# mako443/Text2Pos-CVPR2022

Hardware: AMD Instinct MI355X
Metric: cells+queries encoded/sec and top-k retrieval QPS, 256-pt cells, 12k-cell DB (higher is better)
Workload: dtype f16x3 (fp32 operands split hi+lo into fp16, 3 f16 MFMAs, fp32 accumulate; fp32-class error) for the encoders / f64 MFMA for the ranking

## Files before the change

### include/t2p.h

```cpp
#ifndef T2P_H
#define T2P_H
#include <stddef.h>
#include <stdint.h>

#ifdef __cplusplus
extern "C" {
#endif

#define T2P_ABI_VERSION 31
#define T2P_DEFAULT_CHUNK_OBJECTS 65000
#define T2P_MAX_CHUNK_OBJECTS 65535
#define T2P_TUNING_MASK 0x5
#define T2P_E_ARG (-1)
#define T2P_E_WORKSPACE (-2)
#define T2P_E_UNSUPPORTED (-3)

typedef void* t2p_stream_t;

int t2p_abi_version(void);
const char* t2p_last_error(void);

typedef struct t2p_cell_weights {
    const float* sa_w1[3];
    const float* sa_b1[3];
    const float* sa_w2[3];
    const float* sa_b2[3];
    const float* ga_w1;
    const float* ga_b1;
    const float* ga_w2;
    const float* ga_b2;
    const float* lin1_w;
    const float* lin1_b;
    const float* lin2_w;
    const float* lin2_b;
    const float* pn_w;
    const float* pn_b;
    const float* col_w1;
    const float* col_b1;
    const float* col_w2;
    const float* col_b2;
    const float* pos_w1;
    const float* pos_b1;
    const float* pos_w2;
    const float* pos_b2;
    const float* merge_w;
// ... 221 lines not shown
```

### profiles/tail_rows_census.py

```python
#!/usr/bin/env python
import argparse
import os
import sys

import numpy as np

sys.path.insert(0, os.path.join(os.path.dirname(os.path.abspath(__file__)), ".."))

RADII = (0.2, 0.3, 0.4)
MAX_NBR = 32


def level(pos: np.ndarray, r: float):
    n_d = pos.shape[0]
    n_c = (n_d + 1) // 2
    r2 = np.float32(r) * np.float32(r)
    mind = np.full(n_d, np.inf, dtype=np.float32)
    fps = np.zeros(n_c, dtype=np.int64)
    cnt = np.zeros(n_c, dtype=np.int64)
    cur = 0
    for c in range(n_c):
        fps[c] = cur
        d = pos - pos[cur]
        d2 = (d[:, 0] * d[:, 0] + d[:, 1] * d[:, 1]) + d[:, 2] * d[:, 2]
        cnt[c] = min(int((d2 < r2).sum()), MAX_NBR)
        mind = np.minimum(mind, d2)
        cur = int(np.argmax(mind))
    return fps, cnt


def dedup_hits(pos: np.ndarray, rgb: np.ndarray, fps: np.ndarray, r: float) -> int:
    key = np.concatenate([pos, rgb], axis=1).view(np.uint32)
    _, first = np.unique(key, axis=0, return_index=True)
    orig = np.zeros(pos.shape[0], dtype=bool)
    orig[first] = True
    r2 = np.float32(r) * np.float32(r)
    kept = 0
    for c in fps:
        d = pos - pos[c]
        d2 = (d[:, 0] * d[:, 0] + d[:, 1] * d[:, 1]) + d[:, 2] * d[:, 2]
        hits = np.flatnonzero(d2 < r2)[:MAX_NBR]
        kept += int(orig[hits].sum())
    return kept


def main():
    ap = argparse.ArgumentParser(description=__doc__.split("\n")[0])
    ap.add_argument("--seed", type=int, default=20220002, help="bench.py's object stream")
    ap.add_argument("--objects", type=int, default=3000)
    args = ap.parse_args()
    from importlib import import_module
    S = import_module("text2pos-cvpr2022_amd.synthetic")
    xyz, rgb, _, _ = S.make_objects(args.seed, 0, args.objects)
    n = xyz.shape[0]
    rows = np.zeros(3)
    rows_dedup = 0.0
    with_tail = np.zeros(3)
    tail_cent = np.zeros(3)
    tail_rows = np.zeros(3)
    executed = np.zeros(3)
    cents = np.zeros(3)
    for o in range(n):
        pos = xyz[o].astype(np.float32)
        for l in range(3):
            fps, cnt = level(pos, RADII[l])
            n_c = fps.shape[0]
            tail = (fps == 0) & (np.arange(n_c) > 0)
            all_rows = cnt.sum() + n_c
            t_rows = cnt[tail].sum()
            rows[l] += all_rows
            cents[l] += n_c
            with_tail[l] += tail.any()
            tail_cent[l] += tail.sum()
            tail_rows[l] += t_rows
            executed[l] += all_rows - t_rows + (cnt[0] if tail.any() else 0)
            if l == 0:
                rows_dedup += dedup_hits(pos, rgb[o].astype(np.float32), fps, RADII[0]) + n_c
            pos = pos[fps]
    print(f"{n} objects of seed {args.seed}")
    print("level | rows/object | objects with a tail | tail centroids | tail rows (non-self) | rows/object, tail shared")
    for l in range(3):
        extra = f" ({rows_dedup / n:.0f} after point dedup)" if l == 0 else ""
        print(f"SA{l + 1}   | {rows[l] / n:8.0f}{extra} | {100 * with_tail[l] / n:5.1f} % | {100 * tail_cent[l] / cents[l]:5.1f} % | "
              f"{100 * tail_rows[l] / rows[l]:5.1f} % | {executed[l] / n:8.0f} ({100 * (executed[l] / rows[l] - 1):+.1f} %)")


if __name__ == "__main__":
    main()
```

### text2pos-cvpr2022_amd/csrc/api.hip

```cpp
#include <stdarg.h>
#include <stdlib.h>
#include <string.h>

#include <mutex>
#include <set>
#include <utility>

#include "../../include/t2p.h"
#include "t2p_common.h"

namespace t2p {

static thread_local char g_err[512] = "";

void set_error(const char* fmt, ...) {
    va_list ap;
    va_start(ap, fmt);
    vsnprintf(g_err, sizeof(g_err), fmt, ap);
    va_end(ap);
}

int num_cus() {
    static int cached = 0;
    if (cached == 0) {
// ... 960 lines not shown
    for (int l = 0; l < 3; l++) {
        gt.fps_idx[l] = fps_idx[l];
        gt.nbr[l] = nbr[l];
        gt.cnt[l] = cnt[l];
        gt.rows[l] = nullptr;
        gt.n_rows[l] = nullptr;
        gt.n_dense[l] = g.nd[l];
        gt.n_cent[l] = g.nc[l];
    }
    return launch_sample_group(xyz, n_obj, n_pts, radius_host, gt, (hipStream_t)stream);
}

int t2p_group_rows(const float* xyz, int64_t n_obj, int32_t n_pts, const float* radius_host, int32_t self_loops,
                   uint8_t* const* fps_idx, uint16_t* const* rows, uint16_t* const* n_rows, t2p_stream_t stream) {
    T2P_CHECK_ARG(xyz && radius_host && fps_idx && rows && n_rows, "group_rows: NULL argument");
    Geo g(n_pts);
    GroupTables gt{};
    gt.self_loops = self_loops ? 1 : 0;
    for (int l = 0; l < 3; l++) {
        T2P_CHECK_ARG(fps_idx[l] && rows[l] && n_rows[l], "group_rows: NULL table of level %d", l);
        gt.fps_idx[l] = fps_idx[l];
        gt.rows[l] = rows[l];
        gt.n_rows[l] = n_rows[l];
        gt.n_dense[l] = g.nd[l];
        gt.n_cent[l] = g.nc[l];
    }
    return launch_sample_group(xyz, n_obj, n_pts, radius_host, gt, (hipStream_t)stream);
}

int t2p_group_rows_shared(const float* xyz, int64_t n_obj, int32_t n_pts, const float* radius_host, int32_t self_loops,
                          int32_t share_mask, uint8_t* const* fps_idx, uint16_t* const* rows, uint16_t* const* n_rows,
                          t2p_stream_t stream) {
    T2P_CHECK_ARG(xyz && radius_host && fps_idx && rows && n_rows, "group_rows_shared: NULL argument");
    T2P_CHECK_ARG((share_mask & ~2) == 0, "group_rows_shared: share_mask=%#x (bit 1: SA level 2; no other level has a shared form)", share_mask);
    T2P_CHECK_ARG(share_mask == 0 || n_pts == 256, "group_rows_shared: shared lists exist for 256 points per object (n_pts = %d)", n_pts);
    Geo g(n_pts);
    GroupTables gt{};
    gt.self_loops = self_loops ? 1 : 0;
    for (int l = 0; l < 3; l++) {
        T2P_CHECK_ARG(fps_idx[l] && rows[l] && n_rows[l], "group_rows_shared: NULL table of level %d", l);
        gt.fps_idx[l] = fps_idx[l];
        gt.rows[l] = rows[l];
        gt.n_rows[l] = n_rows[l];
        gt.n_dense[l] = g.nd[l];
        gt.n_cent[l] = g.nc[l];
        gt.share_tail[l] = (share_mask >> l) & 1;
    }
    return launch_sample_group(xyz, n_obj, n_pts, radius_host, gt, (hipStream_t)stream);
}

int t2p_edge_counts(const uint16_t* rows, const uint16_t* n_rows, const int32_t* first_obj, int64_t n_obj, int32_t n_dense,
                    int32_t n_cent, int32_t self_loops, int32_t* counts, t2p_stream_t stream) {
    T2P_CHECK_ARG(n_obj >= 0 && (n_obj == 0 || (rows && n_rows && first_obj && counts)), "edge_counts: NULL argument");
    return launch_edge_counts(rows, n_rows, first_obj, n_obj, n_dense, n_cent, self_loops, counts, (hipStream_t)stream);
}

int t2p_edge_expand(const uint16_t* rows, const uint16_t* n_rows, const int32_t* first_obj, const int32_t* cent_ptr, int64_t n_obj,
                    int32_t n_dense, int32_t n_cent, int32_t self_loops, int32_t* src, int32_t* dst, t2p_stream_t stream) {
    T2P_CHECK_ARG(n_obj >= 0 && (n_obj == 0 || (rows && n_rows && first_obj && cent_ptr)), "edge_expand: NULL argument");
    return launch_edge_expand(rows, n_rows, first_obj, cent_ptr, n_obj, n_dense, n_cent, self_loops, src, dst, (hipStream_t)stream);
}

int t2p_pack_objects(const float* raw_xyz, const float* raw_rgb, const int32_t* obj_ptr, const int32_t* sample_idx,
                     const float* rot_cos_sin, int64_t n_obj, int32_t n_pts, float* xyz, float* rgb, float* center, float* mean_rgb,
                     t2p_stream_t stream) {
    T2P_CHECK_ARG(raw_xyz && raw_rgb && obj_ptr && sample_idx && xyz && rgb && center && mean_rgb, "pack_objects: NULL argument");
    T2P_CHECK_ARG(n_obj >= 0 && n_pts >= 1, "pack_objects: bad sizes");
// ... 53 lines not shown
```

### text2pos-cvpr2022_amd/csrc/sa_points.hip

```cpp
#ifndef T2P_PABL
#define T2P_PABL 0
#endif
#include "t2p_common.h"

namespace t2p {
namespace {

typedef uint32_t u32x4 __attribute__((ext_vector_type(4)));
typedef uint32_t u32x2 __attribute__((ext_vector_type(2)));
typedef float f32x2 __attribute__((ext_vector_type(2)));

#define MFMA16(a, b, c) __builtin_amdgcn_mfma_f32_32x32x16_f16(a, b, c, 0, 0, 0)
#define MFMA8(a, b, c) __builtin_amdgcn_mfma_f32_32x32x8f16(a, b, c, 0, 0, 0)

template <int NW>
struct PtsCfg {
    static constexpr int K = 32, N = 64, NC = 128, ND = 256, GS = 16;
    static constexpr int NT = 64 * NW;
    static constexpr int S16 = K / 16, NTW = N / 32;
    static constexpr int HS = GS / 2, NH = NC / HS;
    static constexpr int MAXR = NC * 33;
    static constexpr int LPR = 64 / HS;
    static constexpr int ACC_BYTES = GS * N * 4;
    static constexpr int PTS_BYTES = ND * 24;
    static constexpr int SELF_BYTES = GS * 24;
    static constexpr int CEN_BYTES = GS * 32;
    static constexpr int RING_BYTES = 4 * 64 * 2;
    static constexpr int WAVE_BYTES = ACC_BYTES + PTS_BYTES + SELF_BYTES + CEN_BYTES + 16 + 64 + RING_BYTES;
    static_assert(WAVE_BYTES % 16 == 0, "16-byte accesses");
    static constexpr size_t lds_bytes() { return (size_t)NW * WAVE_BYTES + 16 + N * 4; }
};

__device__ __forceinline__ float relu1(float v) {
    const int b = __float_as_int(v);
    return __int_as_float(b > 0 ? b : 0);
}
__device__ __forceinline__ void split2(float v0, float v1, uint32_t& hi, uint32_t& lo) {
    const fp16x2 hh = cvt_pk_f16(v0, v1);
    const fp16x2 ll = cvt_pk_f16(sub_half<0>(v0, hh), sub_half<1>(v1, hh));
    hi = __builtin_bit_cast(uint32_t, hh);
    lo = __builtin_bit_cast(uint32_t, ll);
}

template <int NW, int PARTS>
__global__ __launch_bounds__(64 * NW, (NW + 3) / 4) void k_sa_points(SaParams p) {
    using C = PtsCfg<NW>;
    static_assert(PARTS == 1 || (C::NH % PARTS == 0 && C::NH / PARTS >= 3), "a part is a whole number (>= 3: two open + one fetched ahead) of halves");
    constexpr int K = C::K, N = C::N, NC = C::NC;
    extern __shared__ __attribute__((aligned(16))) char lds[];
    const int tid = threadIdx.x, lane = tid & 63;
    const int wave = __builtin_amdgcn_readfirstlane(tid >> 6);
    const int h = lane >> 5, rr = lane & 31;
    const uint32_t acc_off = (uint32_t)(wave * C::WAVE_BYTES);
    const uint32_t pts_off = acc_off + C::ACC_BYTES;
    const uint32_t self_off = pts_off + C::PTS_BYTES;
    const uint32_t cen_off = self_off + C::SELF_BYTES;
    const uint32_t one_off = cen_off + C::CEN_BYTES;
    const uint32_t dst_off = one_off + 16;
    const uint32_t ring_off = dst_off + 64;
    if (lane == 0) *(f32x4*)(lds + one_off) = f32x4{1.f, 0.f, 0.f, 0.f};

    half8 w_hi[C::NTW][C::S16], w_lo[C::NTW][C::S16];
    {
        const uint4* wp = (const uint4*)p.W_x3;
        constexpr int PLANE_U4 = (N / 32) * C::S16 * 64;
#pragma unroll
        for (int nt = 0; nt < C::NTW; nt++)
#pragma unroll
            for (int s = 0; s < C::S16; s++) {
                uint4 pc[2][2];
#pragma unroll
                for (int hp = 0; hp < 2; hp++) {
                    const int kb = 16 * s + 8 * hp;
                    const int half_ = kb / (K / 2), step_ = (kb % (K / 2)) / 8;
                    const int idx = (((nt * C::S16 + step_) * 2 + half_) * 32) + rr;
                    pc[0][hp] = wp[idx];
                    pc[1][hp] = wp[PLANE_U4 + idx];
                }
                const u32x4 vh = h ? u32x4{pc[0][0].z, pc[0][0].w, pc[0][1].z, pc[0][1].w} : u32x4{pc[0][0].x, pc[0][0].y, pc[0][1].x, pc[0][1].y};
                const u32x4 vl = h ? u32x4{pc[1][0].z, pc[1][0].w, pc[1][1].z, pc[1][1].w} : u32x4{pc[1][0].x, pc[1][0].y, pc[1][1].x, pc[1][1].y};
                w_hi[nt][s] = __builtin_bit_cast(half8, vh);
                w_lo[nt][s] = __builtin_bit_cast(half8, vl);
            }
    }
    half4 w1_hi, w1_lo;
    {
// ... 6 lines not shown
        uint32_t hi0, lo0, hi1, lo1;
        split2(wv[0], wv[1], hi0, lo0);
        split2(wv[2], wv[3], hi1, lo1);
        w1_hi = __builtin_bit_cast(half4, u32x2{hi0, hi1});
        w1_lo = __builtin_bit_cast(half4, u32x2{lo0, lo1});
    }
    constexpr f32x16 kZero16 = {0.f, 0.f, 0.f, 0.f, 0.f, 0.f, 0.f, 0.f, 0.f, 0.f, 0.f, 0.f, 0.f, 0.f, 0.f, 0.f};

    const int cr = lane / C::LPR, cs = lane % C::LPR;
    constexpr int NPL = N / C::LPR;
    const uint32_t bias_off = (uint32_t)(NW * C::WAVE_BYTES + 16 + cs * NPL * 4);
    if (tid < N) *(float*)(lds + NW * C::WAVE_BYTES + 16 + tid * 4) = p.bias[tid];

    int gtop = 0;
    const int g_begin = p.bounds_ws[blockIdx.x], g_end = p.bounds_ws[blockIdx.x + 1];
    int* ctr = (int*)(lds + NW * C::WAVE_BYTES);
    if (tid == 0) *ctr = 0;
    __syncthreads();

    f32x4 pout[NPL / 4];
    float* pptr = nullptr;
    bool has_pout = false;
    for (;;) {
        int gi = 0;
        if (lane == 0) gi = atomicAdd(ctr, 1);
        gi = __builtin_amdgcn_readfirstlane(gi);
        const int g = g_begin + (PARTS > 1 ? gi / PARTS : gi);
        if (g >= g_end) break;
        constexpr int HP = C::NH / PARTS;
        const int hs = PARTS > 1 ? (gi % PARTS) * HP : 0;
        const int hend = hs + HP;
        int n = __builtin_amdgcn_readfirstlane((int)p.n_rows[g]);
        const uint16_t* list = p.rows + (int64_t)g * C::MAXR;
        if constexpr (PARTS > 1) {
            auto lower = [&](int target) -> int {
                if (target <= 0 || n <= 0) return 0;
                if (target >= NC) return n;
                const int step = (n + 63) >> 6;
                const int i0 = lane * step;
                const uint32_t c0 = i0 < n ? (((uint32_t)list[i0] >> 8) & 127u) : 255u;
                const unsigned long long ge = __ballot(c0 >= (uint32_t)target);
                const int fl = ge ? (int)__builtin_ctzll(ge) : 64;
                if (fl == 0) return 0;
                int hi = fl * step;
                hi = hi < n ? hi : n;
                const int base = (fl - 1) * step + 1;
                for (int b = base; b < hi; b += 64) {
                    const int i = b + lane;
                    const uint32_t c = i < hi ? (((uint32_t)list[i] >> 8) & 127u) : 255u;
                    const unsigned long long m = __ballot(c >= (uint32_t)target);
                    if (m) return b + (int)__builtin_ctzll(m);
                }
                return hi;
            };
            const int r_lo = __builtin_amdgcn_readfirstlane(lower(hs * C::HS));
            const int r_hi = __builtin_amdgcn_readfirstlane(lower(hend * C::HS));
            list += r_lo;
            n = r_hi - r_lo;
        }
        const int first = __builtin_amdgcn_readfirstlane(p.first[g]);
        const uint32_t sb0 = (uint32_t)(first * C::ND + (g - first) * NC);

        const int nwin = (n + 63) >> 6;
        auto load_win = [&](int w) -> uint32_t {
            int i = w * 64 + lane;
            i = i < n ? i : n - 1;
// ... 3 lines not shown
        auto ring_write = [&](int w, uint32_t v) { *(uint16_t*)(lds + ring_off + (((w & 3) * 64 + lane) * 2)) = (uint16_t)v; };
        auto ring_read = [&](int r) -> uint32_t {
            return (uint32_t) * (const uint16_t*)(lds + ring_off + (((r + rr) & 255) * 2));
        };
        const uint32_t win0 = load_win(0), win1 = load_win(1);
        uint32_t pend = load_win(2);
        int w_loaded = 2;

        typedef float f32x3 __attribute__((ext_vector_type(3)));
        struct Side { f32x3 q, sp, sc; };
        auto fetch_side = [&](int hh) -> Side {
            const int c = hh * C::HS + (lane & (C::HS - 1));
            const float* pc = p.out + ((int64_t)g * NC + c) * (int64_t)p.ldo + N;
            const int64_t ai = (int64_t)sb0 + c;
            return Side{*(const f32x3*)pc, *(const f32x3*)(p.pos_src + ai * 3), *(const f32x3*)(p.feat_src + ai * 3)};
        };
        const Side side0 = fetch_side(hs), side1 = fetch_side(hs + 1);

        {
            const f32x4* px4 = (const f32x4*)(p.pos_src + (int64_t)g * C::ND * 3) + lane * 3;
            const f32x4* pc4 = (const f32x4*)(p.feat_src + (int64_t)g * C::ND * 3) + lane * 3;
            const f32x4 a0 = px4[0], a1 = px4[1], a2 = px4[2];
            const f32x4 c0_ = pc4[0], c1_ = pc4[1], c2_ = pc4[2];
            f32x4* rec = (f32x4*)(lds + pts_off + lane * 96);
            rec[0] = f32x4{c0_[0], c0_[1], c0_[2], a0[0]};
            rec[1] = f32x4{a0[1], a0[2], c0_[3], c1_[0]};
            rec[2] = f32x4{c1_[1], a0[3], a1[0], a1[1]};
            rec[3] = f32x4{c1_[2], c1_[3], c2_[0], a1[2]};
            rec[4] = f32x4{a1[3], a2[0], c2_[1], c2_[2]};
            rec[5] = f32x4{c2_[3], a2[1], a2[2], a2[3]};
        }
        ring_write(0, win0);
        ring_write(1, win1);

        auto flush_out = [&]() {
            if (has_pout) {
#pragma unroll
                for (int q4 = 0; q4 < NPL / 4; q4++) *(f32x4*)(pptr + q4 * 4) = pout[q4];
                has_pout = false;
            }
        };
        auto drain = [&](int hh, bool live) {
            flush_out();
            pptr = p.out + ((int64_t)g * NC + hh * C::HS + cr) * (int64_t)p.ldo + cs * NPL;
            const uint32_t a0 = acc_off + (uint32_t)((((hh & 1) * C::HS + cr) * N + cs * NPL) * 4);
            int top = gtop;
#pragma unroll
            for (int q4 = 0; q4 < NPL / 4; q4++) {
                f32x4 v = f32x4{0.f, 0.f, 0.f, 0.f};
                if (live) {
                    const f32x4 raw = *(const f32x4*)(lds + a0 + q4 * 16);
                    const f32x4 bq = *(const f32x4*)(lds + bias_off + q4 * 16);
#pragma unroll
                    for (int e = 0; e < 4; e++) {
                        const float r = fmaxf(raw[e] + bq[e], 0.f);
                        const int bits = __float_as_int(r);
                        top = bits > top ? bits : top;
                        v[e] = r * p.out_scale;
                    }
                }
                pout[q4] = v;
            }
            has_pout = true;
            gtop = top;
        };
        auto open_half = [&](int hh, const Side& sd) {
            const uint32_t s0 = (uint32_t)((hh & 1) * C::HS);
            if (lane < C::HS) {
                uint2* sp = (uint2*)(lds + self_off + (s0 + lane) * 24);
                sp[0] = uint2{__float_as_uint(sd.sc[0]), __float_as_uint(sd.sc[1])};
                sp[1] = uint2{__float_as_uint(sd.sc[2]), __float_as_uint(sd.sp[0])};
                sp[2] = uint2{__float_as_uint(sd.sp[1]), __float_as_uint(sd.sp[2])};
                f32x4* cp = (f32x4*)(lds + cen_off + (s0 + lane) * 32);
                cp[0] = f32x4{0.f, 0.f, 0.f, sd.q[0]};
                cp[1] = f32x4{sd.q[1], sd.q[2], 0.f, 0.f};
            }
            typedef int i32x4 __attribute__((ext_vector_type(4)));
            const uint32_t a0 = acc_off + (uint32_t)(((s0 + cr) * N + cs * NPL) * 4);
#pragma unroll
            for (int q4 = 0; q4 < NPL / 4; q4++)
                *(i32x4*)(lds + a0 + q4 * 16) = i32x4{(int)0xFF800000, (int)0xFF800000, (int)0xFF800000, (int)0xFF800000};
        };

        open_half(hs, side0);
// ... 17 lines not shown
                }
                if (ho < hd) ho = hd;
                const int want = h0 + 2 < hend ? h0 + 2 : hend;
                while (ho < want) {
                    if (hf != ho) side_n = fetch_side(ho);
                    open_half(ho, side_n);
                    ho++;
                    if (ho < hend) {
                        side_n = fetch_side(ho);
                        hf = ho;
                    }
                }
            }
            if (w_loaded * 64 < r0 + 96 && w_loaded < nwin) {
                ring_write(w_loaded, pend);
                w_loaded++;
                flush_out();
                if (w_loaded < nwin) pend = load_win(w_loaded);
            }
            const uint32_t m = rr < c ? e_cur : (uint32_t)__builtin_amdgcn_readlane((int)e_cur, c - 1);
            const uint32_t src = m & 0xFFu, d = m >> 8;
            const uint32_t dl = d & 15u;
            const uint32_t rec = (d & 0x80u) ? self_off + dl * 24u : pts_off + src * 24u;
            const uint32_t pa0 = rec + (uint32_t)(h * 16), pa1 = h ? one_off : rec + 8u;
            f32x4 pv, cv;
            if constexpr (T2P_PABL & 8) {
                pv = f32x4{(float)pa0, 1.f, 2.f, (float)pa1};
                cv = f32x4{(float)dl, 1.f, 2.f, 3.f};
            } else {
                const f32x2 p0 = *(const f32x2*)(lds + pa0), p1 = *(const f32x2*)(lds + pa1);
                pv = f32x4{p0[0], p0[1], p1[0], p1[1]};
                cv = *(const f32x4*)(lds + cen_off + dl * 32u + (uint32_t)(h * 16));
            }
            *(uint16_t*)(lds + dst_off + rr * 2) = (uint16_t)(dl * (uint32_t)(N * 4));
            uint32_t xh[2], xl[2];
            split2(pv[0] - cv[0], pv[1] - cv[1], xh[0], xl[0]);
            split2(pv[2] - cv[2], pv[3] - cv[3], xh[1], xl[1]);
            const half4 x_hi = __builtin_bit_cast(half4, u32x2{xh[0], xh[1]});
            const half4 x_lo = __builtin_bit_cast(half4, u32x2{xl[0], xl[1]});
            f32x16 hid;
            if constexpr (T2P_PABL & 4) {
#pragma unroll
                for (int e = 0; e < 16; e++) hid[e] = (float)x_hi[e & 3] + (float)x_lo[e & 3];
            } else {
                hid = MFMA8(w1_hi, x_hi, kZero16);
                hid = MFMA8(w1_lo, x_hi, hid);
                hid = MFMA8(w1_hi, x_lo, hid);
            }
            uint2 four[4];
            {
                const uint2* f4 = (const uint2*)(lds + dst_off + h * 8);
                four[0] = f4[0], four[1] = f4[2], four[2] = f4[4], four[3] = f4[6];
            }
            f32x16 acc[C::NTW];
#pragma unroll
            for (int s = 0; s < C::S16; s++) {
                uint32_t nh[4], nl[4];
#pragma unroll
                for (int pr = 0; pr < 4; pr++)
                    split2(relu1(hid[8 * s + 2 * pr]), relu1(hid[8 * s + 2 * pr + 1]), nh[pr], nl[pr]);
                const half8 a_hi = __builtin_bit_cast(half8, u32x4{nh[0], nh[1], nh[2], nh[3]});
                const half8 a_lo = __builtin_bit_cast(half8, u32x4{nl[0], nl[1], nl[2], nl[3]});
                if constexpr (T2P_PABL & 2) {
#pragma unroll
                    for (int nt = 0; nt < C::NTW; nt++)
#pragma unroll
                        for (int e = 0; e < 16; e++) acc[nt][e] = (float)a_hi[e & 7] + (float)a_lo[e & 7];
// ... 15 lines not shown
                }
                static_assert(C::NTW == 2, "the hazard fence below names both result blocks");
                asm volatile("s_nop 15" : "+v"(acc[0]), "+v"(acc[1])::"memory");
#pragma unroll
                for (int nt = 0; nt < C::NTW; nt++)
#pragma unroll
                    for (int e = 0; e < 16; e++)
                        if constexpr (!(T2P_PABL & 1))
                            asm volatile("ds_max_f32 %0, %1 offset:%2" ::"v"(ad[e]), "v"(acc[nt][e]), "n"(nt * 128) : "memory");
                        else
                            asm volatile("; %0 %1" ::"v"(ad[e]), "v"(acc[nt][e]));
            }
            r0 += c;
            e_cur = e_nxt;
        }
        asm volatile("s_waitcnt lgkmcnt(0)" ::: "memory");
        for (; hd < hend; hd++) drain(hd, hd < ho);
        flush_out();
    }
    uint32_t gbits = 0;
    guard_track_bits(gbits, gtop);
    if (p.amax_out != nullptr && lane == 0 && gbits != 0u)
        atomicMax(p.amax_out, __float_as_uint(__uint_as_float(gbits) * p.out_scale));
}

#ifndef T2P_PTS_WAVES
#define T2P_PTS_WAVES 12
#endif
constexpr int kPtsWaves = T2P_PTS_WAVES;
constexpr int kPtsParts = 4;

}

bool sa_points_selected(int H, int Cout, const SaParams& p) {
    return H == 32 && Cout == 64 && p.W_x3 != nullptr && p.wp != nullptr && p.w1 != nullptr;
}

int sa_points_launch_shape(int64_t n_obj, int* tile_rows, int* n_wg) {
    int n = num_cus();
    if (n > 1024) n = 1024;
    if (n > n_obj) n = (int)n_obj;
    *tile_rows = 32;
    *n_wg = n;
    return 0;
}

int launch_sa_points(int H, int Cout, const SaParams& p, hipStream_t st) {
    if (!(H == 32 && Cout == 64 && p.n_cent == 128 && p.n_dense == 256 && p.wp && p.W_x3 && p.w1 && p.b1 && p.feat_src && p.pos_src &&
          p.ld_pos == 3 && p.pos_col0 == 0)) {
        set_error("sa_points: built for SA level 1 (6 -> 32 -> 64, 128 centroids of 256 points [xyz] + [rgb], f16x3)");
        return T2P_E_UNSUPPORTED;
    }
    using C = PtsCfg<kPtsWaves>;
    auto kern = k_sa_points<kPtsWaves, 1>, kern_parts = k_sa_points<kPtsWaves, kPtsParts>;
    T2P_TRY(reserve_lds((const void*)kern, C::lds_bytes(), "sa_points"));
    T2P_TRY(reserve_lds((const void*)kern_parts, C::lds_bytes(), "sa_points"));
    if (p.n_obj <= 0) return 0;
    T2P_CHECK_ARG(p.n_obj < (1 << 22), "sa_points: chunk too large");
    T2P_CHECK_ARG((((uintptr_t)p.pos_src | (uintptr_t)p.feat_src | (uintptr_t)p.out | (uintptr_t)p.W_x3) & 15) == 0 && p.ldo % 4 == 0,
                  "sa_points: points, output rows and weights must be 16-byte aligned");
    int tr, n_wg;
    sa_points_launch_shape(p.n_obj, &tr, &n_wg);
    if (!p.balanced) T2P_TRY(launch_sa_balance(p, tr, n_wg, st));
    ProfScope ps_("ws_edge_sa_k32_n64", st);
    const bool parts = p.n_obj * 2 <= (int64_t)n_wg * kPtsWaves;
    T2P_REPEAT(ps_) hipLaunchKernelGGL(parts ? kern_parts : kern, dim3(n_wg), dim3(C::NT), C::lds_bytes(), st, p);
    T2P_CHECK_LAUNCH("sa_points");
    return 0;
}

}
```

### text2pos-cvpr2022_amd/csrc/sample_group.hip

```cpp
#include "t2p_common.h"

namespace t2p {

#pragma clang fp contract(off)

namespace {

#ifndef T2P_FPS_PK
#define T2P_FPS_PK 1
#endif

constexpr int kMaxPts = 256;
constexpr int kMaxNbr = 32;

__device__ __forceinline__ float dist2(float ax, float ay, float az, float bx, float by, float bz) {
#pragma clang fp contract(off)
    float dx = ax - bx, dy = ay - by, dz = az - bz;
    float xx = dx * dx, yy = dy * dy, zz = dz * dz;
    float s = xx + yy;
    return s + zz;
}

template <int CTRL>
__device__ __forceinline__ int dpp_i(int v) {
// ... 78 lines not shown
            lower = __builtin_amdgcn_mbcnt_hi((uint32_t)(m >> 32), __builtin_amdgcn_mbcnt_lo((uint32_t)m, lower));
            count += __popcll(m);
        }
        int pos = lower;
#pragma unroll
        for (int j = 0; j < PPL; j++) {
            if (hit[j] && pos < kMaxNbr) {
                const int i = lane * PPL + j;
                if (nbr_lds) nbr_lds[c * kMaxNbr + pos] = (uint8_t)i;
                if (rows_out) rows_out[base + pos] = (uint16_t)((c << 8) | i);
            }
            pos += hit[j] ? 1 : 0;
        }
        const int kept = count < kMaxNbr ? count : kMaxNbr;
        if (lane == 0) {
            if (nbr_lds) cnt_lds[c] = (uint8_t)kept;
            if (self_loops && rows_out) rows_out[base + kept] = (uint16_t)(((c | 0x80) << 8) | c);
        }
        base += kept + (self_loops ? 1 : 0);
        if (c + 1 < n_c) {
            const float mx = wave_max_f(bd);
            const unsigned long long tie = __ballot(bd == mx);
            cur = __builtin_amdgcn_readlane(bi, (int)__builtin_ctzll(tie));
        }
    }
    if (rows_out && lane < 4 && base + lane < n_c * (kMaxNbr + 1)) rows_out[base + lane] = 0xFFFF;
    *n_rows_out = base;
    __syncthreads();
}

template <int PPL, bool SHARE = false>
__device__ void level_fast(const float* px, const float* py, const float* pz, int n_c, float r2, uint8_t* sel, float* qx,
                           float* qy, float* qz, uint16_t* __restrict__ rows_out, int self_loops, int* n_rows_out,
                           int tail_code = 0) {
    const int lane = threadIdx.x;
    const int i0 = lane * PPL;
    float x[PPL], y[PPL], z[PPL];
    uint32_t mind[PPL];
#pragma unroll
    for (int j = 0; j < PPL; j++) {
        x[j] = px[i0 + j];
        y[j] = py[i0 + j];
        z[j] = pz[i0 + j];
        mind[j] = 0x7f800000u;
    }
    int cur = 0;
    int base = 0;
    [[maybe_unused]] bool tail_open = false;
    for (int c = 0; c < n_c; c++) {
        const float cx = px[cur], cy = py[cur], cz = pz[cur];
        if (lane == 0) {
            sel[c] = (uint8_t)cur;
            qx[c] = cx;
            qy[c] = cy;
            qz[c] = cz;
        }
        bool tail = false;
        if constexpr (SHARE) {
            tail = c > 0 && cur == 0;
            if (tail && tail_open) {
                if (self_loops && lane == 0) rows_out[(uint32_t)base] = (uint16_t)(((c | 0x80) << 8) | c);
                base += self_loops ? 1 : 0;
                continue;
            }
            tail_open = tail;
        }
        float d[PPL];
        unsigned long long m[PPL];
        if constexpr (T2P_FPS_PK && PPL % 2 == 0) {
            typedef float f32x2 __attribute__((ext_vector_type(2)));
            const f32x2 c2x = {cx, cx}, c2y = {cy, cy}, c2z = {cz, cz};
#pragma unroll
            for (int j = 0; j < PPL; j += 2) {
#pragma clang fp contract(off)
                const f32x2 dx = f32x2{x[j], x[j + 1]} - c2x, dy = f32x2{y[j], y[j + 1]} - c2y, dz = f32x2{z[j], z[j + 1]} - c2z;
                const f32x2 xx = dx * dx, yy = dy * dy, zz = dz * dz;
                const f32x2 sxy = xx + yy;
                const f32x2 dd = sxy + zz;
                d[j] = dd[0];
                d[j + 1] = dd[1];
            }
#pragma unroll
            for (int j = 0; j < PPL; j++) {
                mind[j] = min(mind[j], __float_as_uint(d[j]));
                m[j] = __ballot(d[j] < r2);
            }
        } else {
#pragma unroll
            for (int j = 0; j < PPL; j++) {
                d[j] = dist2(x[j], y[j], z[j], cx, cy, cz);
                mind[j] = min(mind[j], __float_as_uint(d[j]));
                m[j] = __ballot(d[j] < r2);
            }
        }
        int lower = 0, count = 0;
#pragma unroll
        for (int j = 0; j < PPL; j++) {
            lower = __builtin_amdgcn_mbcnt_hi((uint32_t)(m[j] >> 32), __builtin_amdgcn_mbcnt_lo((uint32_t)m[j], lower));
            count += __popcll(m[j]);
        }
        const uint32_t tag = (uint32_t)(tail ? tail_code : c) << 8;
        char* const rows_b = (char*)rows_out;
        if (count <= kMaxNbr) {
            uint32_t off = 2u * (uint32_t)(base + lower);
#pragma unroll
            for (int j = 0; j < PPL; j++) {
                const bool hit = d[j] < r2;
                if (hit) *(uint16_t*)(rows_b + off) = (uint16_t)(tag | (uint32_t)(i0 + j));
                off += hit ? 2u : 0u;
            }
        } else {
            uint32_t pos = (uint32_t)lower;
#pragma unroll
            for (int j = 0; j < PPL; j++) {
                const bool hit = d[j] < r2;
                if (hit && pos < (uint32_t)kMaxNbr) *(uint16_t*)(rows_b + 2u * ((uint32_t)base + pos)) = (uint16_t)(tag | (uint32_t)(i0 + j));
                pos += hit ? 1u : 0u;
            }
        }
        const int kept = count < kMaxNbr ? count : kMaxNbr;
        if (self_loops && lane == 0) rows_out[(uint32_t)(base + kept)] = (uint16_t)(((c | 0x80) << 8) | c);
        base += kept + (self_loops ? 1 : 0);
        if (c + 1 < n_c) {
            uint32_t bd = mind[0];
#pragma unroll
            for (int j = 1; j < PPL; j++) bd = max(bd, mind[j]);
            const uint32_t mx = wave_max_u(bd);
            const unsigned long long tie = __ballot(bd == mx);
            int jb = PPL - 1;
#pragma unroll
            for (int j = PPL - 2; j >= 0; j--) jb = mind[j] == mx ? j : jb;
            cur = __builtin_amdgcn_readlane(i0 + jb, (int)__builtin_ctzll(tie));
        }
    }
    if (lane < 4 && base + lane < n_c * (kMaxNbr + 1)) rows_out[base + lane] = 0xFFFF;
    *n_rows_out = base;
    __syncthreads();
}

__device__ __attribute__((noinline)) void emit_centroid_table(const float* qx, const float* qy, const float* qz, int n_c,
                                                    const float* __restrict__ wp, int H, float* __restrict__ out,
                                                    float* __restrict__ tail, int ld_tail, int tail_col0, int tail_quads,
                                                    int tail_rows) {
    const int lane = threadIdx.x;
    if (tail != nullptr) {
        const int hq = lane % tail_quads;
        for (int c = n_c + lane / tail_quads; c < tail_rows; c += 64 / tail_quads)
            *(f32x4*)(tail + (size_t)c * ld_tail + tail_col0 + hq * 4) =
                hq == 0 ? f32x4{qx[n_c - 1], qy[n_c - 1], qz[n_c - 1], 0.f} : f32x4{0.f, 0.f, 0.f, 0.f};
    }
    if (out == nullptr) {
        if (tail == nullptr) return;
        const int hq = lane % tail_quads;
        for (int c = lane / tail_quads; c < n_c; c += 64 / tail_quads)
            *(f32x4*)(tail + (size_t)c * ld_tail + tail_col0 + hq * 4) =
// ... 66 lines not shown
        if (gt.guard != nullptr) {
            if (gt.rgb != nullptr) {
                const float* col = gt.rgb + o * (int64_t)n_pts * 3;
                for (int i = lane; i < n_pts * 3; i += 64) {
                    const uint32_t b = __float_as_uint(col[i]) & 0x7fffffffu;
                    in_bits = b > in_bits ? b : in_bits;
                }
            }
            guard_publish_bits_above(gt.guard + G_INPUT, in_bits, 0x3f800000u);
        }
        __syncthreads();
        if (gt.A1 != nullptr) {
            const float *w1 = gt.w1, *b1 = gt.b1;
            asm volatile("" : "+s"(w1), "+s"(b1));
            emit_point_table(p0, p0 + kMaxPts, p0 + 2 * kMaxPts, gt.rgb + o * (int64_t)n_pts * 3, n_pts, w1, b1, gt.H1,
                             gt.A1 + o * (int64_t)n_pts * gt.H1);
        }
        float* pin[4][3] = {{p0, p0 + kMaxPts, p0 + 2 * kMaxPts},
                            {p1, p1 + kMaxPts / 2, p1 + kMaxPts},
                            {p2, p2 + kMaxPts / 4, p2 + kMaxPts / 2},
                            {p3, p3 + kMaxPts / 8, p3 + kMaxPts / 4}};
        const float rr[3] = {r0 * r0, r1 * r1, r2 * r2};
#pragma unroll
        for (int l = 0; l < 3; l++) {
            const int n_d = gt.n_dense[l], n_c = gt.n_cent[l];
            if (want_nbr) {
                for (int i = lane; i < n_c * kMaxNbr / 4; i += 64) ((uint32_t*)nbr_lds)[i] = 0u;
            }
            __syncthreads();
            int n_rows = 0;
            uint16_t* g_rows16 = gt.rows[l] ? gt.rows[l] + o * (int64_t)(n_c * (kMaxNbr + 1)) : nullptr;
            if constexpr (FAST) {
                if (l == 0)
                    level_fast<4>(pin[l][0], pin[l][1], pin[l][2], n_c, rr[l], sel_lds, pin[l + 1][0], pin[l + 1][1],
                                  pin[l + 1][2], g_rows16, gt.self_loops, &n_rows);
                else if (l == 1 && gt.share_tail[1])
                    level_fast<2, true>(pin[l][0], pin[l][1], pin[l][2], n_c, rr[l], sel_lds, pin[l + 1][0], pin[l + 1][1],
                                        pin[l + 1][2], g_rows16, gt.self_loops, &n_rows, kSaTailCode);
                else if (l == 1)
                    level_fast<2>(pin[l][0], pin[l][1], pin[l][2], n_c, rr[l], sel_lds, pin[l + 1][0], pin[l + 1][1],
                                  pin[l + 1][2], g_rows16, gt.self_loops, &n_rows);
                else
                    level_fast<1>(pin[l][0], pin[l][1], pin[l][2], n_c, rr[l], sel_lds, pin[l + 1][0], pin[l + 1][1],
                                  pin[l + 1][2], g_rows16, gt.self_loops, &n_rows);
            } else if (n_d > 128)
                level<4>(pin[l][0], pin[l][1], pin[l][2], n_d, n_c, rr[l], sel_lds, pin[l + 1][0], pin[l + 1][1],
                         pin[l + 1][2], nbr_lds, cnt_lds, g_rows16, gt.self_loops, &n_rows);
            else if (n_d > 64)
                level<2>(pin[l][0], pin[l][1], pin[l][2], n_d, n_c, rr[l], sel_lds, pin[l + 1][0], pin[l + 1][1],
                         pin[l + 1][2], nbr_lds, cnt_lds, g_rows16, gt.self_loops, &n_rows);
            else
                level<1>(pin[l][0], pin[l][1], pin[l][2], n_d, n_c, rr[l], sel_lds, pin[l + 1][0], pin[l + 1][1],
                         pin[l + 1][2], nbr_lds, cnt_lds, g_rows16, gt.self_loops, &n_rows);
            if (g_rows16 != nullptr && lane == 0) gt.n_rows[l][o] = (uint16_t)n_rows;
            if (gt.B[l] != nullptr || gt.tail[l] != nullptr) {
                const float* wpl = gt.wp[l];
                asm volatile("" : "+s"(wpl));
                const int t_rows = gt.tail_rows[l] > n_c ? gt.tail_rows[l] : n_c;
                emit_centroid_table(pin[l + 1][0], pin[l + 1][1], pin[l + 1][2], n_c, wpl, gt.H[l],
                                    gt.B[l] ? gt.B[l] + o * (int64_t)n_c * gt.H[l] : nullptr,
                                    gt.tail[l] ? gt.tail[l] + o * (int64_t)t_rows * gt.ld_tail[l] : nullptr, gt.ld_tail[l],
                                    gt.tail_col0[l], l == 2 ? 8 : 1, t_rows);
            }
            uint8_t* g_sel = gt.fps_idx[l] + o * (int64_t)n_c;
            for (int i = lane; i < n_c; i += 64) g_sel[i] = sel_lds[i];
            if (want_nbr) {
                uint8_t* g_nbr = gt.nbr[l] + o * (int64_t)n_c * kMaxNbr;
                uint8_t* g_cnt = gt.cnt[l] + o * (int64_t)n_c;
                for (int i = lane; i < n_c * kMaxNbr / 4; i += 64) ((uint32_t*)g_nbr)[i] = ((const uint32_t*)nbr_lds)[i];
                for (int i = lane; i < n_c; i += 64) g_cnt[i] = cnt_lds[i];
            }
            __syncthreads();
        }
    }
// ... 128 lines not shown
```

### text2pos-cvpr2022_amd/csrc/t2p_common.h

```cpp
#pragma once
#include <hip/hip_runtime.h>
#include <stdint.h>
#include <stdio.h>

namespace t2p {

void set_error(const char* fmt, ...);

#define T2P_E_ARG (-1)
#define T2P_E_WORKSPACE (-2)
#define T2P_E_UNSUPPORTED (-3)

#define T2P_CHECK_ARG(cond, ...)                  \
    do {                                          \
        if (!(cond)) {                            \
            ::t2p::set_error(__VA_ARGS__);        \
            return T2P_E_ARG;                     \
        }                                         \
    } while (0)

#define T2P_CHECK_LAUNCH(name)                                                   \
    do {                                                                         \
        hipError_t e__ = hipGetLastError();                                      \
        if (e__ != hipSuccess) {                                                 \
// ... 213 lines not shown
    const float* A;
    const float* Bc;
    const float* wp;
    const float* W;
    const void* W_x3;
    const float* bias;
    float out_scale;
    float* out;
    int ldo;
    const uint16_t* rows;
    const uint16_t* n_rows;
    const int32_t* first;
    const uint8_t* fps_idx;
    const float* pos_src;
    int ld_pos, pos_col0;
    const float* feat_src;
    const float* w1;
    const float* b1;
    int n_dense, n_cent;
    int64_t n_obj;
    int32_t* prefix_ws;
    int32_t* bounds_ws;
    int balanced;
    uint32_t* amax_out;
    int out_rows;
};
int launch_ws_sa(int H, int C, const SaParams& p, hipStream_t st);
int launch_sa_balance(const SaParams& p, int tile_rows, int n_wg, hipStream_t st);
constexpr int kSaTailCode = 64;
bool sa_rows_selected(int H, int C, const SaParams& p);
int launch_sa_rows(int H, int C, const SaParams& p, hipStream_t st);
int sa_rows_launch_shape(int64_t n_obj, int* tile_rows, int* n_wg);
bool sa_points_selected(int H, int C, const SaParams& p);
int launch_sa_points(int H, int C, const SaParams& p, hipStream_t st);
int sa_points_launch_shape(int64_t n_obj, int* tile_rows, int* n_wg);
bool sa3_selected(int H, int C, const SaParams& p);
int launch_sa3(const SaParams& p, hipStream_t st);
int sa3_launch_shape(int64_t n_obj, int* tile_rows, int* n_wg);
inline bool sa_shares_tail_rows(int l, int H, int C, const SaParams& p, int n_pts, int tuning) {
    return l == 1 && n_pts == 256 && !(tuning & 4) && p.n_dense == 128 && p.n_cent == 64 && sa_rows_selected(H, C, p);
}
int launch_sa_balance_levels(const SaParams p[3], const int H[3], const int C[3], hipStream_t st);

int launch_bilstm_impl(const float* gate_table , const float* whh ,
                       const void* whh_x3 ,
                       float whh_scale, const int32_t* tokens , const int32_t* lengths, int B, int T, int V, int D,
                       float* hdir_ws , float* out ,
                       hipStream_t st);

int launch_lstm_cell_fwd(const float* pre, const float* table, const int32_t* tokens, const int32_t* lengths, int64_t B, int T,
                         int D, int step, int reverse, const float* c_prev, const float* h_prev, float* gates, float* c,
                         float* h, hipStream_t st);
int launch_lstm_cell_bwd(const float* dh_gemm, const float* dh_carry_in, const float* dc_in, const float* gates,
                         const float* c_prev, const float* c, const int32_t* lengths, int64_t B, int D, int step, float* d_pre,
                         float* dc_out, float* dh_carry_out, hipStream_t st);

size_t bn_train_workspace_bytes(int64_t rows, int n_seg, int C);
int launch_bn_relu_train_forward(const float* x, const int32_t* seg_ptr, int n_seg, int64_t rows, int C, const float* gamma,
                                 const float* beta, float eps, int relu, float* y, float* mean, float* invstd,
                                 float* var_unbiased, double* part, hipStream_t st);
int launch_bn_relu_train_backward(const float* dy, const float* x, const float* beta, const int32_t* seg_ptr, int n_seg,
                                  int64_t rows, int C, const float* mean, const float* invstd, const float* gamma, int relu,
                                  float* dx, float* dgamma_seg, float* dbeta_seg, double* part, hipStream_t st);
int launch_edge_feat_fwd(const float* x, const float* pos, const float* pos_c, const int32_t* src, const int32_t* dst, int64_t E,
                         int C, int W, float* out, hipStream_t st);
int launch_edge_feat_bwd(const float* dout, const int32_t* src, int64_t E, int C, int W, float* dx, hipStream_t st);
int launch_pair_feat_fwd(const float* x, const int32_t* tgt, const int32_t* src, int64_t E, int D, float* out, hipStream_t st);
int launch_pair_feat_bwd(const float* dout, const int32_t* tgt, const int32_t* src, int64_t E, int D, float* dx, hipStream_t st);
int launch_segment_mean(const float* x, const int32_t* seg_ptr, int n_seg, int C, float* out, hipStream_t st);
int launch_segment_mean_backward(const float* dout, const int32_t* seg_ptr, int n_seg, int C, float* dx, hipStream_t st);
int launch_rownorm_bwd(const float* x, const float* dy, int64_t n_rows, int dim, float* dx, hipStream_t st);
int launch_segment_max(const float* x, const int32_t* seg_ptr, int n_seg, int C, float* out, int32_t* arg, hipStream_t st);
int launch_segment_max_backward(const float* dout, const int32_t* arg, const int32_t* seg_ptr, int n_seg, int C, float* dx,
// ... 14 lines not shown
```

Baseline: 155,300.

## Share FPS tail rows at SA level 1 to skip duplicate centroid groups

Extends the tail-sharing scheme from SA level 2 to SA level 1. Once farthest-point sampling returns to point 0, the grouping stops and fills the remaining centroids with self-loops only. The SA1 points kernel then finds the tail start from the FPS indices, routes the first tail centroid's accumulation into an extra LDS slot, and max-merges it into every tail row when draining. This removes redundant neighbor-row MLP work for degenerate objects, at the cost of one more accumulator row of LDS per wave and extra drain logic. It only applies in the whole-object kernel variant and is controlled by a new tuning bit.

```diff
diff --git a/include/t2p.h b/include/t2p.h
--- a/include/t2p.h
+++ b/include/t2p.h
@@ -10,7 +10,7 @@
 #define T2P_ABI_VERSION 31
 #define T2P_DEFAULT_CHUNK_OBJECTS 65000
 #define T2P_MAX_CHUNK_OBJECTS 65535
-#define T2P_TUNING_MASK 0x5
+#define T2P_TUNING_MASK 0xD
 #define T2P_E_ARG (-1)
 #define T2P_E_WORKSPACE (-2)
 #define T2P_E_UNSUPPORTED (-3)
diff --git a/profiles/tail_rows_census.py b/profiles/tail_rows_census.py
--- a/profiles/tail_rows_census.py
+++ b/profiles/tail_rows_census.py
@@ -29,18 +29,18 @@
     return fps, cnt
 
 
-def dedup_hits(pos: np.ndarray, rgb: np.ndarray, fps: np.ndarray, r: float) -> int:
+def dedup_hits(pos: np.ndarray, rgb: np.ndarray, fps: np.ndarray, r: float) -> np.ndarray:
     key = np.concatenate([pos, rgb], axis=1).view(np.uint32)
     _, first = np.unique(key, axis=0, return_index=True)
     orig = np.zeros(pos.shape[0], dtype=bool)
     orig[first] = True
     r2 = np.float32(r) * np.float32(r)
-    kept = 0
-    for c in fps:
+    kept = np.zeros(fps.shape[0], dtype=np.int64)
+    for i, c in enumerate(fps):
         d = pos - pos[c]
         d2 = (d[:, 0] * d[:, 0] + d[:, 1] * d[:, 1]) + d[:, 2] * d[:, 2]
         hits = np.flatnonzero(d2 < r2)[:MAX_NBR]
-        kept += int(orig[hits].sum())
+        kept[i] = int(orig[hits].sum())
     return kept
 
 
@@ -55,6 +55,7 @@
     n = xyz.shape[0]
     rows = np.zeros(3)
     rows_dedup = 0.0
+    rows_dedup_shared = 0.0
     with_tail = np.zeros(3)
     tail_cent = np.zeros(3)
     tail_rows = np.zeros(3)
@@ -75,12 +76,15 @@
             tail_rows[l] += t_rows
             executed[l] += all_rows - t_rows + (cnt[0] if tail.any() else 0)
             if l == 0:
-                rows_dedup += dedup_hits(pos, rgb[o].astype(np.float32), fps, RADII[0]) + n_c
+                kept = dedup_hits(pos, rgb[o].astype(np.float32), fps, RADII[0])
+                rows_dedup += kept.sum() + n_c
+                rows_dedup_shared += kept[~tail].sum() + (kept[0] if tail.any() else 0) + n_c
             pos = pos[fps]
     print(f"{n} objects of seed {args.seed}")
     print("level | rows/object | objects with a tail | tail centroids | tail rows (non-self) | rows/object, tail shared")
     for l in range(3):
-        extra = f" ({rows_dedup / n:.0f} after point dedup)" if l == 0 else ""
+        extra = (f" ({rows_dedup / n:.0f} after point dedup, {rows_dedup_shared / n:.0f} with the tail shared: "
+                 f"{100 * (rows_dedup_shared / rows_dedup - 1):+.1f} %)") if l == 0 else ""
         print(f"SA{l + 1}   | {rows[l] / n:8.0f}{extra} | {100 * with_tail[l] / n:5.1f} % | {100 * tail_cent[l] / cents[l]:5.1f} % | "
               f"{100 * tail_rows[l] / rows[l]:5.1f} % | {executed[l] / n:8.0f} ({100 * (executed[l] / rows[l] - 1):+.1f} %)")
 
diff --git a/text2pos-cvpr2022_amd/csrc/api.hip b/text2pos-cvpr2022_amd/csrc/api.hip
--- a/text2pos-cvpr2022_amd/csrc/api.hip
+++ b/text2pos-cvpr2022_amd/csrc/api.hip
@@ -1016,7 +1016,7 @@
                           int32_t share_mask, uint8_t* const* fps_idx, uint16_t* const* rows, uint16_t* const* n_rows,
                           t2p_stream_t stream) {
     T2P_CHECK_ARG(xyz && radius_host && fps_idx && rows && n_rows, "group_rows_shared: NULL argument");
-    T2P_CHECK_ARG((share_mask & ~2) == 0, "group_rows_shared: share_mask=%#x (bit 1: SA level 2; no other level has a shared form)", share_mask);
+    T2P_CHECK_ARG((share_mask & ~3) == 0, "group_rows_shared: share_mask=%#x (bit 0: SA level 1, bit 1: SA level 2; level 3 has no shared form)", share_mask);
     T2P_CHECK_ARG(share_mask == 0 || n_pts == 256, "group_rows_shared: shared lists exist for 256 points per object (n_pts = %d)", n_pts);
     Geo g(n_pts);
     GroupTables gt{};
diff --git a/text2pos-cvpr2022_amd/csrc/sa_points.hip b/text2pos-cvpr2022_amd/csrc/sa_points.hip
--- a/text2pos-cvpr2022_amd/csrc/sa_points.hip
+++ b/text2pos-cvpr2022_amd/csrc/sa_points.hip
@@ -21,7 +21,7 @@
     static constexpr int HS = GS / 2, NH = NC / HS;
     static constexpr int MAXR = NC * 33;
     static constexpr int LPR = 64 / HS;
-    static constexpr int ACC_BYTES = GS * N * 4;
+    static constexpr int ACC_BYTES = (GS + 1) * N * 4;
     static constexpr int PTS_BYTES = ND * 24;
     static constexpr int SELF_BYTES = GS * 24;
     static constexpr int CEN_BYTES = GS * 32;
@@ -52,6 +52,7 @@
     const int wave = __builtin_amdgcn_readfirstlane(tid >> 6);
     const int h = lane >> 5, rr = lane & 31;
     const uint32_t acc_off = (uint32_t)(wave * C::WAVE_BYTES);
+    const uint32_t x_off = acc_off + (uint32_t)(C::GS * N * 4);
     const uint32_t pts_off = acc_off + C::ACC_BYTES;
     const uint32_t self_off = pts_off + C::PTS_BYTES;
     const uint32_t cen_off = self_off + C::SELF_BYTES;
@@ -124,6 +125,8 @@
         const int hend = hs + HP;
         int n = __builtin_amdgcn_readfirstlane((int)p.n_rows[g]);
         const uint16_t* list = p.rows + (int64_t)g * C::MAXR;
+        uint32_t fps2 = 0x0101u;
+        if constexpr (PARTS == 1) fps2 = *(const uint16_t*)(p.fps_idx + (int64_t)g * NC + lane * 2);
         if constexpr (PARTS > 1) {
             auto lower = [&](int target) -> int {
                 if (target <= 0 || n <= 0) return 0;
@@ -193,6 +196,14 @@
         }
         ring_write(0, win0);
         ring_write(1, win1);
+        int t0 = NC;
+        if constexpr (PARTS == 1) {
+            const unsigned long long z0 = __ballot((fps2 & 0xFFu) == 0u && lane > 0), z1 = __ballot((fps2 >> 8) == 0u);
+            const int t_even = z0 ? 2 * (int)__builtin_ctzll(z0) : NC, t_odd = z1 ? 2 * (int)__builtin_ctzll(z1) + 1 : NC;
+            t0 = t_even < t_odd ? t_even : t_odd;
+            *(int*)(lds + x_off + lane * 4) = (int)0xFF800000;
+        }
+        const uint32_t t0x = t0 < NC ? (uint32_t)t0 : 0xFFFFu;
 
         auto flush_out = [&]() {
             if (has_pout) {
@@ -203,14 +214,22 @@
         };
         auto drain = [&](int hh, bool live) {
             flush_out();
+            const bool tail_half = PARTS == 1 && (hh + 1) * C::HS > t0;
+            const bool tail_row = hh * C::HS + cr >= t0;
             pptr = p.out + ((int64_t)g * NC + hh * C::HS + cr) * (int64_t)p.ldo + cs * NPL;
             const uint32_t a0 = acc_off + (uint32_t)((((hh & 1) * C::HS + cr) * N + cs * NPL) * 4);
             int top = gtop;
 #pragma unroll
             for (int q4 = 0; q4 < NPL / 4; q4++) {
                 f32x4 v = f32x4{0.f, 0.f, 0.f, 0.f};
-                if (live) {
-                    const f32x4 raw = *(const f32x4*)(lds + a0 + q4 * 16);
+                if (live || tail_half) {
+                    f32x4 raw = f32x4{-INFINITY, -INFINITY, -INFINITY, -INFINITY};
+                    if (live) raw = *(const f32x4*)(lds + a0 + q4 * 16);
+                    if (tail_half) {
+                        const f32x4 xr = *(const f32x4*)(lds + x_off + (uint32_t)(cs * NPL * 4 + q4 * 16));
+#pragma unroll
+                        for (int e = 0; e < 4; e++) raw[e] = tail_row ? fmaxf(raw[e], xr[e]) : raw[e];
+                    }
                     const f32x4 bq = *(const f32x4*)(lds + bias_off + q4 * 16);
 #pragma unroll
                     for (int e = 0; e < 4; e++) {
@@ -294,7 +313,7 @@
                 pv = f32x4{p0[0], p0[1], p1[0], p1[1]};
                 cv = *(const f32x4*)(lds + cen_off + dl * 32u + (uint32_t)(h * 16));
             }
-            *(uint16_t*)(lds + dst_off + rr * 2) = (uint16_t)(dl * (uint32_t)(N * 4));
+            *(uint16_t*)(lds + dst_off + rr * 2) = (uint16_t)((PARTS == 1 && d == t0x ? (uint32_t)C::GS : dl) * (uint32_t)(N * 4));
             uint32_t xh[2], xl[2];
             split2(pv[0] - cv[0], pv[1] - cv[1], xh[0], xl[0]);
             split2(pv[2] - cv[2], pv[3] - cv[3], xh[1], xl[1]);
@@ -376,6 +395,12 @@
 
 }
 
+bool sa_points_whole_objects(int64_t n_obj) {
+    int tr, n_wg;
+    sa_points_launch_shape(n_obj, &tr, &n_wg);
+    return n_obj * 2 > (int64_t)n_wg * kPtsWaves;
+}
+
 bool sa_points_selected(int H, int Cout, const SaParams& p) {
     return H == 32 && Cout == 64 && p.W_x3 != nullptr && p.wp != nullptr && p.w1 != nullptr;
 }
@@ -390,7 +415,7 @@
 }
 
 int launch_sa_points(int H, int Cout, const SaParams& p, hipStream_t st) {
-    if (!(H == 32 && Cout == 64 && p.n_cent == 128 && p.n_dense == 256 && p.wp && p.W_x3 && p.w1 && p.b1 && p.feat_src && p.pos_src &&
+    if (!(H == 32 && Cout == 64 && p.n_cent == 128 && p.n_dense == 256 && p.wp && p.W_x3 && p.w1 && p.b1 && p.feat_src && p.pos_src && p.fps_idx &&
           p.ld_pos == 3 && p.pos_col0 == 0)) {
         set_error("sa_points: built for SA level 1 (6 -> 32 -> 64, 128 centroids of 256 points [xyz] + [rgb], f16x3)");
         return T2P_E_UNSUPPORTED;
@@ -407,7 +432,7 @@
     sa_points_launch_shape(p.n_obj, &tr, &n_wg);
     if (!p.balanced) T2P_TRY(launch_sa_balance(p, tr, n_wg, st));
     ProfScope ps_("ws_edge_sa_k32_n64", st);
-    const bool parts = p.n_obj * 2 <= (int64_t)n_wg * kPtsWaves;
+    const bool parts = !sa_points_whole_objects(p.n_obj);
     T2P_REPEAT(ps_) hipLaunchKernelGGL(parts ? kern_parts : kern, dim3(n_wg), dim3(C::NT), C::lds_bytes(), st, p);
     T2P_CHECK_LAUNCH("sa_points");
     return 0;
diff --git a/text2pos-cvpr2022_amd/csrc/sample_group.hip b/text2pos-cvpr2022_amd/csrc/sample_group.hip
--- a/text2pos-cvpr2022_amd/csrc/sample_group.hip
+++ b/text2pos-cvpr2022_amd/csrc/sample_group.hip
@@ -134,7 +134,7 @@
 template <int PPL, bool SHARE = false>
 __device__ void level_fast(const float* px, const float* py, const float* pz, int n_c, float r2, uint8_t* sel, float* qx,
                            float* qy, float* qz, uint16_t* __restrict__ rows_out, int self_loops, int* n_rows_out,
-                           int tail_code = 0) {
+                           int share = 0, int tail_code = -1) {
     const int lane = threadIdx.x;
     const int i0 = lane * PPL;
     float x[PPL], y[PPL], z[PPL];
@@ -148,7 +148,6 @@
     }
     int cur = 0;
     int base = 0;
-    [[maybe_unused]] bool tail_open = false;
     for (int c = 0; c < n_c; c++) {
         const float cx = px[cur], cy = py[cur], cz = pz[cur];
         if (lane == 0) {
@@ -158,15 +157,7 @@
             qz[c] = cz;
         }
         bool tail = false;
-        if constexpr (SHARE) {
-            tail = c > 0 && cur == 0;
-            if (tail && tail_open) {
-                if (self_loops && lane == 0) rows_out[(uint32_t)base] = (uint16_t)(((c | 0x80) << 8) | c);
-                base += self_loops ? 1 : 0;
-                continue;
-            }
-            tail_open = tail;
-        }
+        if constexpr (SHARE) tail = share && c > 0 && cur == 0;
         float d[PPL];
         unsigned long long m[PPL];
         if constexpr (T2P_FPS_PK && PPL % 2 == 0) {
@@ -201,7 +192,7 @@
             lower = __builtin_amdgcn_mbcnt_hi((uint32_t)(m[j] >> 32), __builtin_amdgcn_mbcnt_lo((uint32_t)m[j], lower));
             count += __popcll(m[j]);
         }
-        const uint32_t tag = (uint32_t)(tail ? tail_code : c) << 8;
+        const uint32_t tag = (uint32_t)(tail && tail_code >= 0 ? tail_code : c) << 8;
         char* const rows_b = (char*)rows_out;
         if (count <= kMaxNbr) {
             uint32_t off = 2u * (uint32_t)(base + lower);
@@ -223,6 +214,19 @@
         const int kept = count < kMaxNbr ? count : kMaxNbr;
         if (self_loops && lane == 0) rows_out[(uint32_t)(base + kept)] = (uint16_t)(((c | 0x80) << 8) | c);
         base += kept + (self_loops ? 1 : 0);
+        if constexpr (SHARE) {
+            if (tail) {
+                for (int cc = c + 1 + lane; cc < n_c; cc += 64) {
+                    sel[cc] = 0;
+                    qx[cc] = cx;
+                    qy[cc] = cy;
+                    qz[cc] = cz;
+                    if (self_loops) rows_out[(uint32_t)(base + cc - (c + 1))] = (uint16_t)(((cc | 0x80) << 8) | cc);
+                }
+                base += self_loops ? n_c - (c + 1) : 0;
+                break;
+            }
+        }
         if (c + 1 < n_c) {
             uint32_t bd = mind[0];
 #pragma unroll
@@ -355,14 +359,11 @@
             uint16_t* g_rows16 = gt.rows[l] ? gt.rows[l] + o * (int64_t)(n_c * (kMaxNbr + 1)) : nullptr;
             if constexpr (FAST) {
                 if (l == 0)
-                    level_fast<4>(pin[l][0], pin[l][1], pin[l][2], n_c, rr[l], sel_lds, pin[l + 1][0], pin[l + 1][1],
-                                  pin[l + 1][2], g_rows16, gt.self_loops, &n_rows);
-                else if (l == 1 && gt.share_tail[1])
+                    level_fast<4, true>(pin[l][0], pin[l][1], pin[l][2], n_c, rr[l], sel_lds, pin[l + 1][0], pin[l + 1][1],
+                                        pin[l + 1][2], g_rows16, gt.self_loops, &n_rows, gt.share_tail[0], -1);
+                else if (l == 1)
                     level_fast<2, true>(pin[l][0], pin[l][1], pin[l][2], n_c, rr[l], sel_lds, pin[l + 1][0], pin[l + 1][1],
-                                        pin[l + 1][2], g_rows16, gt.self_loops, &n_rows, kSaTailCode);
-                else if (l == 1)
-                    level_fast<2>(pin[l][0], pin[l][1], pin[l][2], n_c, rr[l], sel_lds, pin[l + 1][0], pin[l + 1][1],
-                                  pin[l + 1][2], g_rows16, gt.self_loops, &n_rows);
+                                        pin[l + 1][2], g_rows16, gt.self_loops, &n_rows, gt.share_tail[1], kSaTailCode);
                 else
                     level_fast<1>(pin[l][0], pin[l][1], pin[l][2], n_c, rr[l], sel_lds, pin[l + 1][0], pin[l + 1][1],
                                   pin[l + 1][2], g_rows16, gt.self_loops, &n_rows);
diff --git a/text2pos-cvpr2022_amd/csrc/t2p_common.h b/text2pos-cvpr2022_amd/csrc/t2p_common.h
--- a/text2pos-cvpr2022_amd/csrc/t2p_common.h
+++ b/text2pos-cvpr2022_amd/csrc/t2p_common.h
@@ -269,13 +269,17 @@
 int launch_sa_rows(int H, int C, const SaParams& p, hipStream_t st);
 int sa_rows_launch_shape(int64_t n_obj, int* tile_rows, int* n_wg);
 bool sa_points_selected(int H, int C, const SaParams& p);
+bool sa_points_whole_objects(int64_t n_obj);
 int launch_sa_points(int H, int C, const SaParams& p, hipStream_t st);
 int sa_points_launch_shape(int64_t n_obj, int* tile_rows, int* n_wg);
 bool sa3_selected(int H, int C, const SaParams& p);
 int launch_sa3(const SaParams& p, hipStream_t st);
 int sa3_launch_shape(int64_t n_obj, int* tile_rows, int* n_wg);
 inline bool sa_shares_tail_rows(int l, int H, int C, const SaParams& p, int n_pts, int tuning) {
-    return l == 1 && n_pts == 256 && !(tuning & 4) && p.n_dense == 128 && p.n_cent == 64 && sa_rows_selected(H, C, p);
+    if (n_pts != 256) return false;
+    if (l == 0)
+        return !(tuning & 8) && p.n_dense == 256 && p.n_cent == 128 && sa_points_selected(H, C, p) && sa_points_whole_objects(p.n_obj);
+    return l == 1 && !(tuning & 4) && p.n_dense == 128 && p.n_cent == 64 && sa_rows_selected(H, C, p);
 }
 int launch_sa_balance_levels(const SaParams p[3], const int H[3], const int C[3], hipStream_t st);
 
```

New measurement: 155,800 (median of 2 runs). No clear change (+0.3%).
